# jimmc414/semantic_merge

Measured on AMD Instinct MI355X. Metric: op-log compose+conflict throughput (ops/s), 100M-op logs, 1/2/4/8 GPUs, higher is better.
Workload: dtype u64; 1 GPU; c3: one merge of 100,000,000 ops (100,000,000 per GPU), 1,000,000 symbols, 64 ops/ms, seed 11; n_ops_per_gpu=100000000, n_ops_total=100000000, n_sym=1000000, composed_ops=99989720, conflicts=5140, plan=presorted, parallelism=single GPU

## Files before the change

### include/smx.h

```cpp
#ifndef SMX_H
#define SMX_H

#include <stddef.h>
#include <stdint.h>

#ifdef __cplusplus
extern "C" {
#endif

#define SMX_OK 0
#define SMX_E_ARG (-1)
#define SMX_E_CAPACITY (-2)
#define SMX_E_HIP (-3)
#define SMX_E_WORKSPACE (-4)

#define SMX_KIND_MOVE 0
#define SMX_KIND_RENAME 1
#define SMX_N_KINDS 18
#define SMX_NONE (-1)

typedef struct smx_ops {
  int64_t n_a;
  int64_t n_b;
  int64_t n_sym;
// ... 8 lines not shown
} smx_ops;

typedef struct smx_compose_out {
  int32_t* order;
  int32_t* addr;
  int32_t* file;
  int32_t* ctx;
  int32_t* conflicts;
  int64_t conflict_cap;
  int64_t* counts;
} smx_compose_out;

int smx_compose_workspace_bytes(int64_t n_a, int64_t n_b, int64_t n_sym, size_t* bytes);

int smx_compose(const smx_ops* ops, const smx_compose_out* out, void* workspace,
                size_t workspace_bytes, void* stream);

int smx_compose_async(const smx_ops* ops, const smx_compose_out* out, void* workspace,
                      size_t workspace_bytes, void* stream);
int smx_compose_finish(const smx_ops* ops, const smx_compose_out* out, void* workspace,
                       size_t workspace_bytes, void* stream);

int smx_release_graphs(void* stream);

#define SMX_PLAN_PRESORTED 0
#define SMX_PLAN_SEGMENTED 1
#define SMX_PLAN_RADIX 2
#define SMX_PLAN_RADIX_LO 3
#define SMX_PLAN_PRESORTED_WIDE 4
#define SMX_PLAN_SMALL 5
int smx_last_plan(void);

int64_t smx_set_small_limit(int64_t n);

typedef struct smx_batch {
  int64_t n_merges, n_total, n_sym;
  const int64_t* off;
  const int64_t* n_a;
  const uint8_t* kind; const uint64_t* ts, *oid_hi, *oid_lo;
  const uint32_t* sym; const int32_t* v0, *v1;
  int32_t* order, *addr, *file, *ctx;
  int32_t* conflicts; const int64_t* conf_off;
  int64_t* counts;
  int32_t grid_cap;
} smx_batch;
int smx_compose_batch_workspace_bytes(int64_t n_merges, size_t* bytes);
int smx_compose_batch(const smx_batch* b, void* workspace, size_t workspace_bytes, void* stream);

typedef struct smx_batch_shared {
  int64_t n_merges, n_total, n_sym;
  int64_t n_shared;
  const int64_t* off;
  const uint8_t* kind; const uint64_t* ts, *oid_hi, *oid_lo;
  const uint32_t* sym; const int32_t* v0, *v1;
  int32_t* order, *addr, *file, *ctx;
  int32_t* conflicts; const int64_t* conf_off;
  int64_t* counts;
  int32_t grid_cap;
  int32_t shared_is_b;
} smx_batch_shared;
int smx_compose_batch_shared_workspace_bytes(int64_t n_merges, size_t* bytes);
int smx_compose_batch_shared(const smx_batch_shared* b, void* workspace, size_t workspace_bytes, void* stream);

#define SMX_BATCH_LARGE 1u
int smx_compose_batch_ex_workspace_bytes(int64_t n_merges, int64_t n_total, uint32_t flags, size_t* bytes);
int smx_compose_batch_shared_ex_workspace_bytes(int64_t n_merges, int64_t n_total, int64_t n_shared, uint32_t flags,
// ... 138 lines not shown
```

### semantic_merge_amd/_abi.py

```python
from __future__ import annotations

import ctypes as C

c_i64p = C.POINTER(C.c_int64)


class SmxOps(C.Structure):
    _fields_ = [
        ("n_a", C.c_int64),
        ("n_b", C.c_int64),
        ("n_sym", C.c_int64),
        ("kind", C.c_void_p),
        ("ts", C.c_void_p),
        ("oid_hi", C.c_void_p),
        ("oid_lo", C.c_void_p),
        ("sym", C.c_void_p),
        ("v0", C.c_void_p),
        ("v1", C.c_void_p),
        ("b_gap", C.c_int64),
    ]


class SmxComposeOut(C.Structure):
    _fields_ = [
# ... 177 lines not shown
        ("list", C.c_void_p),
        ("op", C.c_void_p),
        ("value", C.c_void_p),
        ("anchor", C.c_void_p),
        ("t", C.c_void_p),
        ("author", C.c_void_p),
        ("opid_hi", C.c_void_p),
        ("opid_lo", C.c_void_p),
    ]


class SmxRgaOut(C.Structure):
    _fields_ = [
        ("out_value", C.c_void_p),
        ("out_src", C.c_void_p),
        ("out_offsets", C.c_void_p),
        ("counts", C.c_void_p),
        ("out_tomb", C.c_void_p),
    ]


RGA_GROUPED = 1
SCREEN_LARGE = 1
BATCH_LARGE = 1

EXPORTS = (
    "smx_compose_workspace_bytes",
    "smx_compose",
    "smx_compose_async",
    "smx_compose_finish",
    "smx_release_graphs",
    "smx_last_plan",
    "smx_set_small_limit",
    "smx_compose_batch_workspace_bytes",
    "smx_compose_batch",
    "smx_compose_batch_shared_workspace_bytes",
    "smx_compose_batch_shared",
    "smx_compose_batch_ex_workspace_bytes",
    "smx_compose_batch_ex",
    "smx_compose_batch_shared_ex_workspace_bytes",
    "smx_compose_batch_shared_ex",
    "smx_compose_pairs_workspace_bytes",
    "smx_compose_pairs",
    "smx_screen_workspace_bytes",
    "smx_screen",
    "smx_screen_ex_workspace_bytes",
    "smx_screen_ex",
    "smx_screen_candidates_workspace_bytes",
    "smx_screen_candidates",
    "smx_shard_step",
    "smx_shard_range_info",
    "smx_set_profiling",
    "smx_set_profiling_stages",
    "smx_stage_times",
    "smx_stage_name",
    "smx_reset_stage_times",
    "smx_rga_workspace_bytes",
    "smx_rga_replay",
    "smx_rga_replay_ex",
    "smx_last_error",
    "smx_version",
)


def declare(lib: C.CDLL) -> C.CDLL:
    lib.smx_compose_workspace_bytes.argtypes = [C.c_int64, C.c_int64, C.c_int64,
                                                C.POINTER(C.c_size_t)]
    lib.smx_compose_workspace_bytes.restype = C.c_int
    lib.smx_compose.argtypes = [C.POINTER(SmxOps), C.POINTER(SmxComposeOut), C.c_void_p,
                                C.c_size_t, C.c_void_p]
    lib.smx_compose.restype = C.c_int
    for f in ("smx_compose_async", "smx_compose_finish"):
        getattr(lib, f).argtypes = lib.smx_compose.argtypes
        getattr(lib, f).restype = C.c_int
    lib.smx_release_graphs.argtypes = [C.c_void_p]
    lib.smx_release_graphs.restype = C.c_int
    lib.smx_last_plan.argtypes = []
    lib.smx_last_plan.restype = C.c_int
    lib.smx_set_small_limit.argtypes = [C.c_int64]
    lib.smx_set_small_limit.restype = C.c_int64
    if hasattr(lib, "smx_compose_batch"):
        lib.smx_compose_batch_workspace_bytes.argtypes = [C.c_int64, C.POINTER(C.c_size_t)]
        lib.smx_compose_batch_workspace_bytes.restype = C.c_int
        lib.smx_compose_batch.argtypes = [C.POINTER(SmxBatch), C.c_void_p, C.c_size_t, C.c_void_p]
        lib.smx_compose_batch.restype = C.c_int
    if hasattr(lib, "smx_compose_batch_shared"):
        lib.smx_compose_batch_shared_workspace_bytes.argtypes = [C.c_int64, C.POINTER(C.c_size_t)]
        lib.smx_compose_batch_shared_workspace_bytes.restype = C.c_int
        lib.smx_compose_batch_shared.argtypes = [C.POINTER(SmxBatchShared), C.c_void_p, C.c_size_t, C.c_void_p]
        lib.smx_compose_batch_shared.restype = C.c_int
    if hasattr(lib, "smx_compose_batch_ex"):
        lib.smx_compose_batch_ex_workspace_bytes.argtypes = [C.c_int64, C.c_int64, C.c_uint32, C.POINTER(C.c_size_t)]
        lib.smx_compose_batch_ex_workspace_bytes.restype = C.c_int
        lib.smx_compose_batch_ex.argtypes = [C.POINTER(SmxBatch), C.c_void_p, C.c_size_t, C.c_uint32, C.c_void_p]
        lib.smx_compose_batch_ex.restype = C.c_int
        lib.smx_compose_batch_shared_ex_workspace_bytes.argtypes = [C.c_int64, C.c_int64, C.c_int64, C.c_uint32,
                                                                    C.POINTER(C.c_size_t)]
        lib.smx_compose_batch_shared_ex_workspace_bytes.restype = C.c_int
        lib.smx_compose_batch_shared_ex.argtypes = [C.POINTER(SmxBatchShared), C.c_void_p, C.c_size_t, C.c_uint32,
                                                    C.c_void_p]
        lib.smx_compose_batch_shared_ex.restype = C.c_int
    if hasattr(lib, "smx_compose_pairs"):
        lib.smx_compose_pairs_workspace_bytes.argtypes = [C.c_int64, C.c_int64, C.c_int64, C.c_uint32,
                                                          C.POINTER(C.c_size_t)]
        lib.smx_compose_pairs_workspace_bytes.restype = C.c_int
        lib.smx_compose_pairs.argtypes = [C.POINTER(SmxPairs), C.c_void_p, C.c_size_t, C.c_uint32, C.c_void_p]
        lib.smx_compose_pairs.restype = C.c_int
    if hasattr(lib, "smx_screen"):
        lib.smx_screen_workspace_bytes.argtypes = [C.c_int64, C.c_int64, C.c_int64, C.POINTER(C.c_size_t)]
        lib.smx_screen_workspace_bytes.restype = C.c_int
        lib.smx_screen.argtypes = [C.POINTER(SmxScreen), C.c_void_p, C.c_size_t, C.c_void_p]
        lib.smx_screen.restype = C.c_int
    if hasattr(lib, "smx_screen_ex"):
# ... 41 lines not shown
```

### semantic_merge_amd/csrc/smx_compose.hip

```cpp
#include <algorithm>
#include <atomic>
#include <cstring>
#include <mutex>
#include <string>
#include <vector>

#include "smx_sort.h"
#include "smx_window.h"
#include "smx_small.h"
#include "smx_tables.h"


#include "smx_prof.h"

#include "smx_plan.h"
#include "smx_walk.h"

#include "smx_emit.h"


struct Layout {
  size_t off[64];
  size_t total;
};
// ... 243 lines not shown
  if (!tb_geometry(C, &width, &nbk)) return SMX_OK;
  TbArgs A = tb_args(C);
  A.width = (u32)width;
  A.nbk = (u32)nbk;
  A.keep_skip = 1u;
  hipLaunchKernelGGL(k_tb_scatter, dim3((int)SMX_CEIL_DIV((u64)C.n, (u64)TB_TILE)), dim3(TB_NT), 0, C.st, A,
                     C.ws<u32>(B_TBHIST), C.ws<u32>(B_REC));
  HIP_TRY(hipGetLastError());
  return SMX_OK;
}

static int launch_tables(const Ctx& C, void* part_tab, u32 tag, int tagbits, bool* bucketed,
                         bool prescattered = false) {
  hipStream_t st = C.st;
  const i64 n = C.n;
  int4* fin = C.ws<int4>(B_FIN);
  *bucketed = false;
  const i64 n_sym = C.n_sym;
  TbArgs A = tb_args(C);
  u64 width, nbk;
  if (tb_geometry(C, &width, &nbk)) {
    *bucketed = true;
    A.width = (u32)width;
    A.nbk = (u32)nbk;
    const int nblk = (int)SMX_CEIL_DIV((u64)n, (u64)TB_TILE);
    u32* lst = C.ws<u32>(B_TBHIST);
    u32* rec = C.ws<u32>(B_REC);
    if (prescattered) {
      A.keep_skip = 1u;
      hipLaunchKernelGGL(k_tb_unskip, dim3(1024), dim3(BLOCK), 0, st, A, lst, rec, C.ws<u32>(B_SKIPLIST));
    } else {
      hipLaunchKernelGGL(k_tb_scatter, dim3(nblk), dim3(TB_NT), 0, st, A, lst, rec);
    }
    hipLaunchKernelGGL(k_tb_reduce, dim3(nbk), dim3(TBR_NT), 0, st, A, lst, rec, n_sym, fin,
                       PartTab{part_tab, tag, tagbits, C.ws<ComposeMeta>(B_META)});
  } else {
    u32* tabA = C.ws<u32>(B_TABA);
    u32* tabF = C.ws<u32>(B_TABF);
    u32* tabR = C.ws<u32>(B_TABR);
    int rc;
    if ((rc = zero_async(tabA, (size_t)n_sym * 4, st)) || (rc = zero_async(tabF, (size_t)n_sym * 4, st)) ||
        (rc = zero_async(tabR, (size_t)n_sym * 4, st)))
      return rc;
    hipLaunchKernelGGL(k_tab_atomic, dim3(grid_for(n)), dim3(BLOCK), 0, st, A, tabA, tabF, tabR);
    hipLaunchKernelGGL(k_finalize, dim3(grid_for(n_sym)), dim3(BLOCK), 0, st, A, tabA, tabF, tabR, n_sym, fin,
                       PartTab{part_tab, tag, tagbits, C.ws<ComposeMeta>(B_META)});
  }
  HIP_TRY(hipGetLastError());
  return SMX_OK;
}

static int launch_emit(const Ctx& C, bool packable, const smx_shard* sh) {
  hipStream_t st = C.st;
  ComposeMeta* meta = C.ws<ComposeMeta>(B_META);
  const i64 n = C.n;
  EmitArgs E{C.ws<i32>(B_TSRC), C.ws<u32>(B_TSYM), C.ws<u64>(B_SKIPBITS), C.ws<u32>(B_SKIPLIST),
             C.ws<int4>(B_FIN), meta, (u64)n, (u32)(C.n_sym - 1), packable ? 1 : 0, (u64)C.na, C.src_a,
             C.src_b, C.src_map, C.out->order, C.out->addr, C.out->file, C.out->ctx, C.out->counts, sh ? 0 : 1,
             sh ? nullptr : C.hrec, C.hseq};
  const i64 ewaves = SMX_CEIL_DIV(n, (i64)EMIT_WT);
  const bool al16 = ((uintptr_t)C.out->order | (uintptr_t)C.out->addr | (uintptr_t)C.out->file |
                     (uintptr_t)C.out->ctx) % 16 == 0;
  if (al16)
    hipLaunchKernelGGL(k_emit4, dim3(SMX_CEIL_DIV(ewaves, (i64)NWAVES)), dim3(BLOCK), 0, st, E);
  else
    hipLaunchKernelGGL(k_emit, dim3(SMX_CEIL_DIV(ewaves, (i64)NWAVES)), dim3(BLOCK), 0, st, E);
  HIP_TRY(hipGetLastError());
  return SMX_OK;
}

#if SMX_DIAG
static int knob(const char* name, int dflt) {
  const char* v = getenv(name);
  return v && *v ? atoi(v) : dflt;
}
#else
static constexpr int knob(const char*, int dflt) { return dflt; }
#endif

struct SideStream {
  std::mutex mu;
  int dev = -1;
  hipStream_t caller = nullptr;
  hipStream_t s = nullptr;
  hipEvent_t fork = nullptr, join = nullptr;
};
#define SIDE_MAX 256
static std::mutex g_side_mu;
static SideStream* g_side[SIDE_MAX];
static int g_nside = 0;

static int side_stream(hipStream_t caller, SideStream** out) {
  *out = nullptr;
  int dev = 0;
  HIP_TRY(hipGetDevice(&dev));
  std::lock_guard<std::mutex> g(g_side_mu);
  for (int i = 0; i < g_nside; ++i)
    if (g_side[i]->dev == dev && g_side[i]->caller == caller) {
      *out = g_side[i];
      return SMX_OK;
    }
  if (g_nside == SIDE_MAX) return SMX_OK;
  SideStream* S = new SideStream;
  S->dev = dev;
  S->caller = caller;
  int ncu = 0;
  HIP_TRY(hipDeviceGetAttribute(&ncu, hipDeviceAttributeMultiprocessorCount, dev));
  const int k = knob("SMX_SIDE_CUS", 0);
  if (k > 0 && k < ncu) {
    std::vector<uint32_t> mask((size_t)(ncu + 31) / 32, 0u);
    for (int i = 0; i < k; ++i) mask[(size_t)i / 32] |= 1u << (i % 32);
    HIP_TRY(hipExtStreamCreateWithCUMask(&S->s, (uint32_t)mask.size(), mask.data()));
  } else {
    HIP_TRY(hipStreamCreateWithFlags(&S->s, hipStreamNonBlocking));
  }
  const unsigned evf = hipEventDisableTiming | hipEventDisableSystemFence;
  HIP_TRY(hipEventCreateWithFlags(&S->fork, evf));
  HIP_TRY(hipEventCreateWithFlags(&S->join, evf));
  g_side[g_nside++] = S;
  *out = S;
  return SMX_OK;
}

#ifndef SMX_TB_UNSKIP_MAXN
#define SMX_TB_UNSKIP_MAXN (1 << 22)
#endif
#ifndef SMX_TB_OVERLAP_MIN
#define SMX_TB_OVERLAP_MIN (1 << 18)
#endif

static int launch_tail(const Ctx& C) {
  u64 width, nbk;
  const bool geo = tb_geometry(C, &width, &nbk);
  SideStream* S = nullptr;
  if (geo && C.n >= SMX_TB_OVERLAP_MIN && !knob("SMX_TB_SERIAL", 0)) {
    int rc = side_stream(C.st, &S);
    if (rc) return rc;
  }
  std::unique_lock<std::mutex> own;
  int rc;
  hipStream_t st = C.st;
  TbArgs A{};
  u32* lst = C.ws<u32>(B_TBHIST);
  u32* rec = C.ws<u32>(B_REC);
  if (S) {
    own = std::unique_lock<std::mutex>(S->mu);
    A = tb_args(C);
    A.width = (u32)width;
    A.nbk = (u32)nbk;
    A.keep_skip = C.n <= SMX_TB_UNSKIP_MAXN ? 2u : 1u;
    const int nblk = (int)SMX_CEIL_DIV((u64)C.n, (u64)TB_TILE);
    HIP_TRY(hipEventRecord(S->fork, st));
    HIP_TRY(hipStreamWaitEvent(S->s, S->fork, 0));
    hipLaunchKernelGGL(k_tb_scatter, dim3(nblk), dim3(TB_NT), 0, S->s, A, lst, rec);
    HIP_TRY(hipGetLastError());
    HIP_TRY(hipEventRecord(S->join, S->s));
  }
  C.tm->begin(ST_WALK);
  if ((rc = launch_walk(C, nullptr))) {
    if (S) (void)hipStreamWaitEvent(st, S->join, 0);
    return rc;
  }
  C.tm->end(ST_WALK);
  if (S) HIP_TRY(hipStreamWaitEvent(st, S->join, 0));
  C.tm->begin(ST_TABLES);
  bool bucketed = true;
  if (S) {
    if (A.keep_skip == 1u)
      hipLaunchKernelGGL(k_tb_unskip, dim3(1024), dim3(BLOCK), 0, st, A, lst, rec, C.ws<u32>(B_SKIPLIST));
    hipLaunchKernelGGL(k_tb_reduce, dim3(nbk), dim3(TBR_NT), 0, st, A, lst, rec, C.n_sym, C.ws<int4>(B_FIN),
                       PartTab{nullptr, 0u, 0, nullptr});
    HIP_TRY(hipGetLastError());
  } else if ((rc = launch_tables(C, nullptr, 0, 0, &bucketed))) {
    return rc;
  }
  C.tm->end(ST_TABLES);
  C.tm->begin(ST_EMIT);
  if ((rc = launch_emit(C, bucketed, nullptr))) return rc;
  C.tm->end(ST_EMIT);
  return SMX_OK;
}


struct EarlyFail {
  u32* flag_host = nullptr;
  u32* flag_dev = nullptr;
  hipEvent_t ev = nullptr;
};
enum WinLevel { WL_NORMAL, WL_WIDE };
static i64 level_cap(int lv) { return lv == WL_WIDE ? WF_WIDE_CAP : WF_CAP; }
static int first_level(const Ctx& C) { return knob("SMX_FIRST_WIDE", 0) ? WL_WIDE : WL_NORMAL; }
static i64 first_tgt(const Ctx& C) {
  return knob("SMX_WIN_TGT", first_level(C) == WL_WIDE ? WF_WIDE_CAP : WIN_TGT);
}

template <int CAP, int NT, bool DBG, bool MAP, bool RUNS>
static void launch_window_f(const WinArgs& P, hipStream_t st) {
  hipLaunchKernelGGL((k_window_f<CAP, NT, DBG, MAP, RUNS>), dim3(P.W), dim3(NT), 0, st, P);
}
template <int CAP, int NT>
static void launch_window_level(const WinArgs& P, hipStream_t st) {
  if (P.src_map) launch_window_f<CAP, NT, false, true, true>(P, st);
  else launch_window_f<CAP, NT, false, false, true>(P, st);
}

static int launch_presorted_windows(const Ctx& C, i64 W, i64 CM, int level) {
  const bool wide = level == WL_WIDE;
  hipStream_t st = C.st;
  WinArgs P = win_args(C);
  P.cpre = C.ws<u32>(B_CCNT);
  P.CM = CM;
// ... 564 lines not shown
  return entry(ops,
               [&] { return compose_async_impl(ops, out, workspace, workspace_bytes, (hipStream_t)stream, false); });
}

extern "C" int smx_compose_finish(const smx_ops* ops, const smx_compose_out* out, void* workspace,
                                  size_t workspace_bytes, void* stream) {
  return entry(ops, [&] { return compose_finish_impl(ops, out, workspace, workspace_bytes, (hipStream_t)stream); });
}

extern "C" int smx_compose(const smx_ops* ops, const smx_compose_out* out, void* workspace,
                           size_t workspace_bytes, void* stream) {
  return entry(ops, [&] {
    EarlyVerdict ev;
    if (SmallRec* r = small_rec()) {
      ev.hrec = r->d;
      ev.hrec_host = r->h;
      ev.hseq = ++r->seq;
    }
    const int rc = compose_async_impl(ops, out, workspace, workspace_bytes, (hipStream_t)stream, true, &ev);
    return rc ? rc : compose_finish_impl(ops, out, workspace, workspace_bytes, (hipStream_t)stream, &ev);
  });
}

extern "C" int smx_last_plan(void) { return g_plan; }

#ifdef SMALL_STAMPS
extern "C" int smx_diag_small_stamps(uint64_t* host16) {
  HIP_TRY(hipDeviceSynchronize());
  HIP_TRY(hipMemcpyFromSymbol(host16, HIP_SYMBOL(g_small_stamp), 16 * sizeof(u64)));
  return SMX_OK;
}
#endif

extern "C" int64_t smx_set_small_limit(int64_t n) {
  const int64_t v = n < 0 ? 0 : n > SMALL_N ? SMALL_N : n;
  return g_small_max.exchange(v);
}


extern "C" const char* smx_version(void) { return "smx 0.2 gfx950"; }
```

### semantic_merge_amd/csrc/smx_emit.h

```cpp
#pragma once

struct EmitArgs {
  const i32* tsrc;
  const u32* tsym;
  const u64* skipbits;
  const u32* skiplist;
  const int4* fin;
  const ComposeMeta* meta;
  u64 n;
  u32 smax;
  int allow_pack;
  u64 na_loc;
  i64 src_a, src_b;
  const i32* src_map;
  i32* out_order;
  i32* out_addr;
  i32* out_file;
  i32* out_ctx;
  i64* counts;
  int status_none;
  u64* hrec;
  u64 hseq;
};

#define NTLD(p) __builtin_nontemporal_load(p)
#define NTST(v, p) __builtin_nontemporal_store((v), (p))
#ifndef EMIT_WT
#define EMIT_WT 1024
#endif
#ifndef EMIT_B
#define EMIT_B 8
#endif
static_assert(EMIT_WT % (WAVE * EMIT_B) == 0, "a wave's output range is whole batches of steps");

__global__ void __launch_bounds__(BLOCK) k_emit(EmitArgs E) {
  const ComposeMeta* M = E.meta;
  if (blockIdx.x == 0 && threadIdx.x == 0) {
    const bool bad = M->bad_sym != 0;
    E.counts[0] = bad ? -1 : M->f_fail ? -2 : (M->n_move_none && E.status_none) ? -3 : (i64)(E.n - M->n_skip);
    E.counts[1] = bad ? -1 : (i64)M->n_conf;
    if (E.hrec) *E.hrec = E.hseq << 1 | ((bad || M->f_fail || (M->n_move_none && M->kcnt[KMOVE])) ? 1u : 0u);
  }
  if (M->f_fail | M->bad_sym) return;
  const u64 nskip = M->n_skip;
  const u64 nmv = min(M->kcnt[KMOVE], E.n);
  const u64 nP = E.n - nmv;
  const u64 nR = min(M->kcnt[KREN], nP);
  const u64 nout = E.n - nskip, nRk = nR - nskip;
  auto gsrc = [&](i32 j) -> i32 {
    if (E.src_map) return E.src_map[j];
    return (u64)j < E.na_loc ? (i32)(E.src_a + j) : (i32)(E.src_b + ((i64)j - (i64)E.na_loc));
  };
  const FinPack FP = fin_pack_of(M->vbits, E.allow_pack != 0);
  const int lane = threadIdx.x & (WAVE - 1);
  const u64 w0 = (((u64)blockIdx.x * BLOCK + threadIdx.x) / WAVE) * EMIT_WT;
// ... 40 lines not shown
    for (int j = 0; j < EMIT_B; ++j) {
      src[j] = NTLD(&E.tsrc[pp[j]]);
      sy[j] = min(NTLD(&E.tsym[pp[j]]), E.smax);
    }
    int4 F[EMIT_B];
    if (FP.packed) {
      u64 x[EMIT_B];
#pragma unroll
      for (int j = 0; j < EMIT_B; ++j) x[j] = fin_word(FP, E.fin, sy[j]);
#pragma unroll
      for (int j = 0; j < EMIT_B; ++j) F[j] = fin_decode(FP, x[j]);
    } else {
#pragma unroll
      for (int j = 0; j < EMIT_B; ++j) F[j] = E.fin[sy[j]];
    }
#pragma unroll
    for (int j = 0; j < EMIT_B; ++j) {
      const u64 o = ob + (u64)j * WAVE + lane;
      if (o >= nmv && o < nout) {
        const bool ren = o - nmv < nRk;
        NTST(gsrc(src[j]), &E.out_order[o]);
        NTST(F[j].x, &E.out_addr[o]);
        NTST(F[j].y, &E.out_file[o]);
        NTST(ren ? -1 : F[j].z, &E.out_ctx[o]);
      }
    }
  }
}

#define EMIT4_STEPS (EMIT_WT / (4 * WAVE))
typedef u32 ev4u __attribute__((ext_vector_type(4)));
typedef i32 ev4i __attribute__((ext_vector_type(4)));
typedef ev4u __attribute__((aligned(4))) ev4u_a4;
__global__ void __launch_bounds__(BLOCK) k_emit4(EmitArgs E) {
  const ComposeMeta* M = E.meta;
  if (blockIdx.x == 0 && threadIdx.x == 0) {
    const bool bad = M->bad_sym != 0;
    E.counts[0] = bad ? -1 : M->f_fail ? -2 : (M->n_move_none && E.status_none) ? -3 : (i64)(E.n - M->n_skip);
    E.counts[1] = bad ? -1 : (i64)M->n_conf;
    if (E.hrec) *E.hrec = E.hseq << 1 | ((bad || M->f_fail || (M->n_move_none && M->kcnt[KMOVE])) ? 1u : 0u);
  }
  if (M->f_fail | M->bad_sym) return;
  const u64 nskip = M->n_skip;
  const u64 nmv = min(M->kcnt[KMOVE], E.n);
  const u64 nP = E.n - nmv;
  const u64 nR = min(M->kcnt[KREN], nP);
  const u64 nout = E.n - nskip, nRk = nR - nskip;
  auto gsrc = [&](i32 j) -> i32 {
    if (E.src_map) return E.src_map[j];
    return (u64)j < E.na_loc ? (i32)(E.src_a + j) : (i32)(E.src_b + ((i64)j - (i64)E.na_loc));
  };
  const FinPack FP = fin_pack_of(M->vbits, E.allow_pack != 0);
  const int lane = threadIdx.x & (WAVE - 1);
  const u64 w0 = (((u64)blockIdx.x * BLOCK + threadIdx.x) / WAVE) * EMIT_WT;
  if (w0 + EMIT_WT <= nmv || w0 >= nout || nP == 0) return;
  u64 kk = 0;
  {
    const u64 o0 = w0 > nmv ? w0 - nmv : 0;
    if (o0 < nRk) {
      u64 lo = 0, hi = nskip;
      while (lo < hi) {
        const u64 mid = (lo + hi) >> 1;
        if ((u64)E.skiplist[mid] - mid < o0) lo = mid + 1;
        else hi = mid;
      }
      kk = lo;
    }
  }
  u64 pp[EMIT4_STEPS][4];
  bool vec[EMIT4_STEPS];
#pragma unroll
  for (int j = 0; j < EMIT4_STEPS; ++j) {
    const u64 b = w0 + (u64)j * 4 * WAVE;
    const u64 o = b + 4 * (u64)lane;
    u64 add[4] = {0, 0, 0, 0};
    const u64 k0 = kk;
    if (b + 4 * WAVE > nmv && (b > nmv ? b - nmv : 0) < nRk) {
      const u64 ohi = b + 4 * WAVE - 1 - nmv;
      while (kk < nskip) {
        const u64 sj = (u64)(u32)__builtin_amdgcn_readfirstlane((int)E.skiplist[kk]) - kk;
        if (sj > ohi) break;
#pragma unroll
        for (int u = 0; u < 4; ++u) add[u] += (o + u >= nmv ? o + u - nmv : 0) >= sj;
        ++kk;
      }
    }
#pragma unroll
    for (int u = 0; u < 4; ++u) {
      const u64 ou = o + u;
      const u64 op = ou >= nmv ? ou - nmv : 0;
      const bool ok = ou >= nmv && ou < nout;
      pp[j][u] = !ok ? 0 : (op < nRk ? op + k0 + add[u] : op + nskip);
    }
    vec[j] = o >= nmv && o + 3 < nout && pp[j][3] == pp[j][0] + 3;
  }
  i32 src[EMIT4_STEPS][4];
  u32 sy[EMIT4_STEPS][4];
#pragma unroll
  for (int j = 0; j < EMIT4_STEPS; ++j) {
    if (vec[j]) {
      const ev4u s4 = __builtin_nontemporal_load(reinterpret_cast<const ev4u_a4*>(&E.tsrc[pp[j][0]]));
      const ev4u y4 = __builtin_nontemporal_load(reinterpret_cast<const ev4u_a4*>(&E.tsym[pp[j][0]]));
      src[j][0] = (i32)s4.x, src[j][1] = (i32)s4.y, src[j][2] = (i32)s4.z, src[j][3] = (i32)s4.w;
      sy[j][0] = y4.x, sy[j][1] = y4.y, sy[j][2] = y4.z, sy[j][3] = y4.w;
    } else {
#pragma unroll
      for (int u = 0; u < 4; ++u) {
        src[j][u] = NTLD(&E.tsrc[pp[j][u]]);
        sy[j][u] = NTLD(&E.tsym[pp[j][u]]);
      }
    }
#pragma unroll
    for (int u = 0; u < 4; ++u) sy[j][u] = min(sy[j][u], E.smax);
  }
#pragma unroll
  for (int j = 0; j < EMIT4_STEPS; ++j) {
    int4 F[4];
    if (FP.packed) {
      u64 x[4];
#pragma unroll
      for (int u = 0; u < 4; ++u) x[u] = fin_word(FP, E.fin, sy[j][u]);
#pragma unroll
      for (int u = 0; u < 4; ++u) F[u] = fin_decode(FP, x[u]);
    } else {
#pragma unroll
      for (int u = 0; u < 4; ++u) F[u] = E.fin[sy[j][u]];
    }
    const u64 o = w0 + (u64)j * 4 * WAVE + 4 * (u64)lane;
    i32 vo[4], va[4], vf[4], vc[4];
#pragma unroll
    for (int u = 0; u < 4; ++u) {
      const bool ren = o + u >= nmv && o + u - nmv < nRk;
      vo[u] = gsrc(src[j][u]);
      va[u] = F[u].x;
      vf[u] = F[u].y;
      vc[u] = ren ? -1 : F[u].z;
    }
    if (o >= nmv && o + 3 < nout) {
      NTST((ev4i{vo[0], vo[1], vo[2], vo[3]}), reinterpret_cast<ev4i*>(&E.out_order[o]));
      NTST((ev4i{va[0], va[1], va[2], va[3]}), reinterpret_cast<ev4i*>(&E.out_addr[o]));
      NTST((ev4i{vf[0], vf[1], vf[2], vf[3]}), reinterpret_cast<ev4i*>(&E.out_file[o]));
      NTST((ev4i{vc[0], vc[1], vc[2], vc[3]}), reinterpret_cast<ev4i*>(&E.out_ctx[o]));
    } else {
#pragma unroll
      for (int u = 0; u < 4; ++u) {
        if (o + u >= nmv && o + u < nout) {
          E.out_order[o + u] = vo[u];
          E.out_addr[o + u] = va[u];
          E.out_file[o + u] = vf[u];
          E.out_ctx[o + u] = vc[u];
        }
      }
    }
  }
}

__global__ void k_mv_init(const u32* __restrict__ msym, u64 nMv, u64* __restrict__ keys, u32* __restrict__ vals) {
  for (u64 j = (u64)blockIdx.x * BLOCK + threadIdx.x; j < nMv; j += (u64)gridDim.x * BLOCK) {
    keys[j] = msym[j] & SYM_MASK;
    vals[j] = (u32)j;
  }
}

__global__ void k_mv_fix(const u64* __restrict__ keys, const u32* __restrict__ vals, u64 nMv,
                         const u32* __restrict__ msym, const u64* __restrict__ mvpre, u64 n_sym,
                         i32* __restrict__ out_addr, i32* __restrict__ out_file) {
  for (u64 j = (u64)blockIdx.x * BLOCK + threadIdx.x; j < nMv; j += (u64)gridDim.x * BLOCK) {
    if (j != 0 && keys[j - 1] == keys[j]) continue;
    i32 ra = -1, rf = -1;
    if (mvpre && keys[j] < n_sym) {
      const u64 pa = mvpre[keys[j]], pf = mvpre[n_sym + keys[j]];
      if (pa) ra = (i32)(u32)pa - 1;
      if (pf) rf = (i32)(u32)pf - 1;
    }
    for (u64 i = j; i < nMv && keys[i] == keys[j]; ++i) {
      const u32 T = vals[i];
      const u32 f = msym[T];
      if (f & MS_HAS_A) ra = out_addr[T];
      else out_addr[T] = ra;
      if (f & MS_HAS_F) rf = out_file[T];
      else out_file[T] = rf;
    }
  }
}
```

### semantic_merge_amd/csrc/smx_tables.h

```cpp
#pragma once

#include "smx_scan.h"

#define TB_WIDTH 4096
#define TB_MAXBK 1024
#ifndef TB_NT
#define TB_NT 1024
#endif
#define TB_NW (TB_NT / WAVE)
#ifndef TB_ITEMS
#define TB_ITEMS 16
#endif
#ifndef TB_NBK_TGT
#define TB_NBK_TGT 256
#endif
#define TB_TILE (TB_NT * TB_ITEMS)
#define REC_IB (TB_TILE <= (1 << 14) ? 14 : 15)
static_assert(TB_TILE <= (1 << 15), "tile-relative record index is at most 15 bits");
#define REC_IMASK ((1u << REC_IB) - 1u)
#define REC_HAS_A (1u << (REC_IB + 12))
#define REC_HAS_F (1u << (REC_IB + 13))

struct TbArgs {
  const u32* msym;
// ... 167 lines not shown

#define TBR_NT 1024
#ifndef TBR_TK
#define TBR_TK 16
#endif
#ifndef TBR_U
#define TBR_U 2
#endif

struct PartTab {
  void* p;
  u32 tag;
  int tagbits;
  ComposeMeta* meta;
  __device__ __forceinline__ void put(i64 n_sym, i64 s, int va, int vf, int vc) const {
    if (tagbits == 0) {
      u64* part = (u64*)p;
      const u64 tg = (u64)tag << 32;
      part[s] = va >= 0 ? tg | (u32)(va + 1) : 0ull;
      part[n_sym + s] = vf >= 0 ? tg | (u32)(vf + 1) : 0ull;
      part[2 * n_sym + s] = vc >= 0 ? tg | (u32)(vc + 1) : 0ull;
      return;
    }
    u32* part = (u32*)p;
    const u32 vb = 31u - (u32)tagbits, tg = tag << vb, lim = 1u << vb;
    const u32 a1 = (u32)(va + 1), f1 = (u32)(vf + 1), c1 = (u32)(vc + 1);
    if ((a1 | f1 | c1) >= lim) meta->tab_over = 1;
    part[s] = va >= 0 ? tg | (a1 & (lim - 1)) : 0u;
    part[n_sym + s] = vf >= 0 ? tg | (f1 & (lim - 1)) : 0u;
    part[2 * n_sym + s] = vc >= 0 ? tg | (c1 & (lim - 1)) : 0u;
  }
};

__global__ void __launch_bounds__(TBR_NT) k_tb_reduce(TbArgs A0, const u32* __restrict__ lst,
                                                      const u32* __restrict__ rec, i64 n_sym,
                                                      int4* __restrict__ fin, PartTab part) {
  const FinPack FP = fin_pack_of(A0.meta->vbits, true);
  __shared__ u32 tA[TB_WIDTH], tF[TB_WIDTH], tC[TB_WIDTH];
  const TbArgs A = tb_load(A0);
  const u32 b = (u32)xcd_item(blockIdx.x, gridDim.x);
  for (u32 i = threadIdx.x; i < A.width; i += TBR_NT) tA[i] = tF[i] = tC[i] = 0;
  __syncthreads();
  auto put = [&](u32 q, u64 rb) {
    const u32 r1 = (u32)(rb + (q & REC_IMASK)) + 1u;
    const u32 ls = (q >> REC_IB) & 0xfffu;
    if ((u64)(r1 - 1) < A.nMv) {
      if (q & REC_HAS_A) atomicMax(&tA[ls], r1);
      if (q & REC_HAS_F) atomicMax(&tF[ls], r1);
    } else if (A.keep_skip != 2u || !tb_skipped(A, (u64)(r1 - 1) - A.nMv)) {
      atomicMax(&tC[ls], r1);
    }
  };
  const u64 nrec = A.nMv + A.nR;
  const int nt = nrec ? (int)SMX_CEIL_DIV(nrec, (u64)TB_TILE) : 0;
  const int lane = threadIdx.x & (WAVE - 1), wv = threadIdx.x / WAVE;
  const u32 nb1 = A.nbk + 1;
  constexpr int NW = TBR_NT / WAVE;
  auto bounds = [&](int t0, u32* lo, u32* hi) {
    *lo = *hi = 0;
    if (lane < TBR_TK && t0 + lane < nt) {
      const u32* lt = lst + (u64)(t0 + lane) * nb1;
      *lo = lt[b];
      *hi = lt[b + 1];
    }
  };
  u32 lo_n = 0, hi_n = 0;
  bounds(wv * TBR_TK, &lo_n, &hi_n);
  for (int t0 = wv * TBR_TK; t0 < nt; t0 += NW * TBR_TK) {
    const u32 lo = lo_n, hi = hi_n;
    u32 q[TBR_TK][TBR_U];
#pragma unroll
    for (int k = 0; k < TBR_TK; ++k) {
      const u32 lk = __builtin_amdgcn_readlane(lo, k), hk = __builtin_amdgcn_readlane(hi, k);
      const u64 rb = (u64)(t0 + k) * TB_TILE;
#pragma unroll
      for (int u = 0; u < TBR_U; ++u) {
        const u32 i = lk + (u32)lane + (u32)(u * WAVE);
        q[k][u] = i < hk ? __builtin_nontemporal_load(&rec[rb + i]) : ~0u;
      }
    }
    bounds(t0 + NW * TBR_TK, &lo_n, &hi_n);
#pragma unroll
    for (int k = 0; k < TBR_TK; ++k)
#pragma unroll
      for (int u = 0; u < TBR_U; ++u)
        if (q[k][u] != ~0u) put(q[k][u], (u64)(t0 + k) * TB_TILE);
#pragma unroll
    for (int k = 0; k < TBR_TK; ++k) {
      const u32 lk = __builtin_amdgcn_readlane(lo, k), hk = __builtin_amdgcn_readlane(hi, k);
      const u64 rb = (u64)(t0 + k) * TB_TILE;
      for (u32 i = lk + TBR_U * WAVE + (u32)lane; i < hk; i += WAVE) {
        const u32 x = rec[rb + i];
        if (x != REC_DEAD) put(x, rb);
      }
    }
  }
  __syncthreads();
  const u32 s0 = b * A.width;
  for (u32 i = threadIdx.x; i < A.width && (i64)(s0 + i) < n_sym; i += TBR_NT) {
    const u32 a = tA[i], f = tF[i], c = tC[i];
    const int va = a ? A.mv_addr[a - 1] : -1, vf = f ? A.mv_file[f - 1] : -1;
    const int vc = c ? A.Rstr[(u64)(c - 1) - A.nMv] : -1;
    if (part.p) part.put(n_sym, s0 + i, va, vf, vc);
    else fin_put(FP, fin, s0 + i, va, vf, vc);
  }
}

__global__ void k_tab_atomic(TbArgs A0, u32* __restrict__ tabA, u32* __restrict__ tabF, u32* __restrict__ tabR) {
  const TbArgs A = tb_load(A0);
  const u64 nrec = A.nMv + A.nR;
  for (u64 r = (u64)blockIdx.x * BLOCK + threadIdx.x; r < nrec; r += (u64)gridDim.x * BLOCK) {
    u32 s, fl;
    if (!tb_record(A, r, &s, &fl)) continue;
    const u32 r1 = (u32)r + 1u;
    if (r < A.nMv) {
      if (fl & REC_HAS_A) atomicMax(&tabA[s], r1);
      if (fl & REC_HAS_F) atomicMax(&tabF[s], r1);
    } else {
      atomicMax(&tabR[s], r1);
    }
  }
}

__global__ void k_finalize(TbArgs A0, const u32* __restrict__ tabA, const u32* __restrict__ tabF,
                           const u32* __restrict__ tabR, i64 n_sym, int4* __restrict__ fin, PartTab part) {
  const TbArgs A = tb_load(A0);
  for (i64 s = (i64)blockIdx.x * BLOCK + threadIdx.x; s < n_sym; s += (i64)gridDim.x * BLOCK) {
    const u32 a = tabA[s], f = tabF[s], c = tabR[s];
    const int va = a ? A.mv_addr[a - 1] : -1, vf = f ? A.mv_file[f - 1] : -1;
    const int vc = c ? A.Rstr[(u64)(c - 1) - A.nMv] : -1;
    if (part.p) part.put(n_sym, s, va, vf, vc);
    else fin[s] = make_int4(va, vf, vc, 0);
  }
}
```

Baseline: 42.64 billion ops/s.

## Split tail reduce into move and rename phases overlapped with emit

For large merges, the table reduce is split in two. The move-table part runs on the side stream right after scatter and writes a packed addr/file table. The rename part is fused into one kernel that also emits the rename output range, and a second emit kernel handles the remaining range. The aim is to overlap reduce work with emit and shorten the serial tail. The cost is an extra packed table pass, re-reading the move table in the rename phase, and more kernel launches.

```diff
diff --git a/include/smx.h b/include/smx.h
--- a/include/smx.h
+++ b/include/smx.h
@@ -64,6 +64,8 @@
 int smx_last_plan(void);
 
 int64_t smx_set_small_limit(int64_t n);
+
+int64_t smx_set_tail_split_min(int64_t n);
 
 typedef struct smx_batch {
   int64_t n_merges, n_total, n_sym;
diff --git a/semantic_merge_amd/_abi.py b/semantic_merge_amd/_abi.py
--- a/semantic_merge_amd/_abi.py
+++ b/semantic_merge_amd/_abi.py
@@ -233,6 +233,7 @@
     "smx_release_graphs",
     "smx_last_plan",
     "smx_set_small_limit",
+    "smx_set_tail_split_min",
     "smx_compose_batch_workspace_bytes",
     "smx_compose_batch",
     "smx_compose_batch_shared_workspace_bytes",
@@ -280,6 +281,9 @@
     lib.smx_last_plan.restype = C.c_int
     lib.smx_set_small_limit.argtypes = [C.c_int64]
     lib.smx_set_small_limit.restype = C.c_int64
+    if hasattr(lib, "smx_set_tail_split_min"):
+        lib.smx_set_tail_split_min.argtypes = [C.c_int64]
+        lib.smx_set_tail_split_min.restype = C.c_int64
     if hasattr(lib, "smx_compose_batch"):
         lib.smx_compose_batch_workspace_bytes.argtypes = [C.c_int64, C.POINTER(C.c_size_t)]
         lib.smx_compose_batch_workspace_bytes.restype = C.c_int
diff --git a/semantic_merge_amd/csrc/smx_compose.hip b/semantic_merge_amd/csrc/smx_compose.hip
--- a/semantic_merge_amd/csrc/smx_compose.hip
+++ b/semantic_merge_amd/csrc/smx_compose.hip
@@ -299,8 +299,8 @@
     } else {
       hipLaunchKernelGGL(k_tb_scatter, dim3(nblk), dim3(TB_NT), 0, st, A, lst, rec);
     }
-    hipLaunchKernelGGL(k_tb_reduce, dim3(nbk), dim3(TBR_NT), 0, st, A, lst, rec, n_sym, fin,
-                       PartTab{part_tab, tag, tagbits, C.ws<ComposeMeta>(B_META)});
+    hipLaunchKernelGGL(k_tb_reduce<TBM_ALL>, dim3(nbk), dim3(TBR_NT), 0, st, A, lst, rec, n_sym, fin,
+                       (void*)nullptr, PartTab{part_tab, tag, tagbits, C.ws<ComposeMeta>(B_META)});
   } else {
     u32* tabA = C.ws<u32>(B_TABA);
     u32* tabF = C.ws<u32>(B_TABF);
@@ -317,19 +317,26 @@
   return SMX_OK;
 }
 
+static void* af_table(const Ctx& C) { return C.ws<void>(B_TABA); }
+
+static EmitArgs emit_args(const Ctx& C, bool packable, const smx_shard* sh) {
+  return EmitArgs{C.ws<i32>(B_TSRC), C.ws<u32>(B_TSYM), C.ws<u64>(B_SKIPBITS), C.ws<u32>(B_SKIPLIST),
+                  C.ws<int4>(B_FIN), C.ws<ComposeMeta>(B_META), (u64)C.n, (u32)(C.n_sym - 1), packable ? 1 : 0,
+                  (u64)C.na, C.src_a, C.src_b, C.src_map, C.out->order, C.out->addr, C.out->file, C.out->ctx,
+                  C.out->counts, sh ? 0 : 1, sh ? nullptr : C.hrec, C.hseq, nullptr};
+}
+
+static bool emit_aligned(const Ctx& C) {
+  return ((uintptr_t)C.out->order | (uintptr_t)C.out->addr | (uintptr_t)C.out->file | (uintptr_t)C.out->ctx) % 16 ==
+         0;
+}
+
 static int launch_emit(const Ctx& C, bool packable, const smx_shard* sh) {
   hipStream_t st = C.st;
-  ComposeMeta* meta = C.ws<ComposeMeta>(B_META);
-  const i64 n = C.n;
-  EmitArgs E{C.ws<i32>(B_TSRC), C.ws<u32>(B_TSYM), C.ws<u64>(B_SKIPBITS), C.ws<u32>(B_SKIPLIST),
-             C.ws<int4>(B_FIN), meta, (u64)n, (u32)(C.n_sym - 1), packable ? 1 : 0, (u64)C.na, C.src_a,
-             C.src_b, C.src_map, C.out->order, C.out->addr, C.out->file, C.out->ctx, C.out->counts, sh ? 0 : 1,
-             sh ? nullptr : C.hrec, C.hseq};
-  const i64 ewaves = SMX_CEIL_DIV(n, (i64)EMIT_WT);
-  const bool al16 = ((uintptr_t)C.out->order | (uintptr_t)C.out->addr | (uintptr_t)C.out->file |
-                     (uintptr_t)C.out->ctx) % 16 == 0;
-  if (al16)
-    hipLaunchKernelGGL(k_emit4, dim3(SMX_CEIL_DIV(ewaves, (i64)NWAVES)), dim3(BLOCK), 0, st, E);
+  const EmitArgs E = emit_args(C, packable, sh);
+  const i64 ewaves = SMX_CEIL_DIV(C.n, (i64)EMIT_WT);
+  if (emit_aligned(C))
+    hipLaunchKernelGGL(k_emit4<EP_ALL>, dim3(SMX_CEIL_DIV(ewaves, (i64)NWAVES)), dim3(BLOCK), 0, st, E);
   else
     hipLaunchKernelGGL(k_emit, dim3(SMX_CEIL_DIV(ewaves, (i64)NWAVES)), dim3(BLOCK), 0, st, E);
   HIP_TRY(hipGetLastError());
@@ -396,6 +403,11 @@
 #define SMX_TB_OVERLAP_MIN (1 << 18)
 #endif
 
+#ifndef SMX_TB_SPLIT_MIN
+#define SMX_TB_SPLIT_MIN (1 << 23)
+#endif
+static std::atomic<int64_t> g_split_min{SMX_TB_SPLIT_MIN};
+
 static int launch_tail(const Ctx& C) {
   u64 width, nbk;
   const bool geo = tb_geometry(C, &width, &nbk);
@@ -404,6 +416,7 @@
     int rc = side_stream(C.st, &S);
     if (rc) return rc;
   }
+  const bool split = S && C.n >= g_split_min.load() && emit_aligned(C);
   std::unique_lock<std::mutex> own;
   int rc;
   hipStream_t st = C.st;
@@ -420,6 +433,9 @@
     HIP_TRY(hipEventRecord(S->fork, st));
     HIP_TRY(hipStreamWaitEvent(S->s, S->fork, 0));
     hipLaunchKernelGGL(k_tb_scatter, dim3(nblk), dim3(TB_NT), 0, S->s, A, lst, rec);
+    if (split)
+      hipLaunchKernelGGL(k_tb_reduce<TBM_MOVES>, dim3(nbk), dim3(TBR_NT), 0, S->s, A, lst, rec, C.n_sym,
+                         (int4*)nullptr, af_table(C), PartTab{nullptr, 0u, 0, nullptr});
     HIP_TRY(hipGetLastError());
     HIP_TRY(hipEventRecord(S->join, S->s));
   }
@@ -435,15 +451,26 @@
   if (S) {
     if (A.keep_skip == 1u)
       hipLaunchKernelGGL(k_tb_unskip, dim3(1024), dim3(BLOCK), 0, st, A, lst, rec, C.ws<u32>(B_SKIPLIST));
-    hipLaunchKernelGGL(k_tb_reduce, dim3(nbk), dim3(TBR_NT), 0, st, A, lst, rec, C.n_sym, C.ws<int4>(B_FIN),
-                       PartTab{nullptr, 0u, 0, nullptr});
+    if (!split)
+      hipLaunchKernelGGL(k_tb_reduce<TBM_ALL>, dim3(nbk), dim3(TBR_NT), 0, st, A, lst, rec, C.n_sym,
+                         C.ws<int4>(B_FIN), (void*)nullptr, PartTab{nullptr, 0u, 0, nullptr});
     HIP_TRY(hipGetLastError());
   } else if ((rc = launch_tables(C, nullptr, 0, 0, &bucketed))) {
     return rc;
   }
   C.tm->end(ST_TABLES);
   C.tm->begin(ST_EMIT);
-  if ((rc = launch_emit(C, bucketed, nullptr))) return rc;
+  if (split) {
+    EmitArgs E = emit_args(C, true, nullptr);
+    E.af = af_table(C);
+    const i64 ewaves = SMX_CEIL_DIV(C.n, (i64)EMIT_WT);
+    hipLaunchKernelGGL(k_emit4_ren_reduce, dim3((u32)nbk + (u32)SMX_CEIL_DIV(ewaves, (i64)(EMITA_NT / WAVE))),
+                       dim3(EMITA_NT), 0, st, E, A, lst, rec, C.n_sym, C.ws<int4>(B_FIN), af_table(C));
+    hipLaunchKernelGGL(k_emit4<EP_REST>, dim3(SMX_CEIL_DIV(ewaves, (i64)NWAVES)), dim3(BLOCK), 0, st, E);
+    HIP_TRY(hipGetLastError());
+  } else if ((rc = launch_emit(C, bucketed, nullptr))) {
+    return rc;
+  }
   C.tm->end(ST_EMIT);
   return SMX_OK;
 }
@@ -1074,6 +1101,8 @@
 }
 #endif
 
+extern "C" int64_t smx_set_tail_split_min(int64_t n) { return g_split_min.exchange(n < 0 ? SMX_TB_SPLIT_MIN : n); }
+
 extern "C" int64_t smx_set_small_limit(int64_t n) {
   const int64_t v = n < 0 ? 0 : n > SMALL_N ? SMALL_N : n;
   return g_small_max.exchange(v);
diff --git a/semantic_merge_amd/csrc/smx_emit.h b/semantic_merge_amd/csrc/smx_emit.h
--- a/semantic_merge_amd/csrc/smx_emit.h
+++ b/semantic_merge_amd/csrc/smx_emit.h
@@ -21,6 +21,7 @@
   int status_none;
   u64* hrec;
   u64 hseq;
+  const void* af;
 };
 
 #define NTLD(p) __builtin_nontemporal_load(p)
@@ -127,14 +128,20 @@
 typedef u32 ev4u __attribute__((ext_vector_type(4)));
 typedef i32 ev4i __attribute__((ext_vector_type(4)));
 typedef ev4u __attribute__((aligned(4))) ev4u_a4;
-__global__ void __launch_bounds__(BLOCK) k_emit4(EmitArgs E) {
+__device__ __forceinline__ void emit_counts(const EmitArgs& E) {
   const ComposeMeta* M = E.meta;
-  if (blockIdx.x == 0 && threadIdx.x == 0) {
-    const bool bad = M->bad_sym != 0;
-    E.counts[0] = bad ? -1 : M->f_fail ? -2 : (M->n_move_none && E.status_none) ? -3 : (i64)(E.n - M->n_skip);
-    E.counts[1] = bad ? -1 : (i64)M->n_conf;
-    if (E.hrec) *E.hrec = E.hseq << 1 | ((bad || M->f_fail || (M->n_move_none && M->kcnt[KMOVE])) ? 1u : 0u);
-  }
+  const bool bad = M->bad_sym != 0;
+  E.counts[0] = bad ? -1 : M->f_fail ? -2 : (M->n_move_none && E.status_none) ? -3 : (i64)(E.n - M->n_skip);
+  E.counts[1] = bad ? -1 : (i64)M->n_conf;
+  if (E.hrec) *E.hrec = E.hseq << 1 | ((bad || M->f_fail || (M->n_move_none && M->kcnt[KMOVE])) ? 1u : 0u);
+}
+
+#define EP_ALL 0
+#define EP_REN 1
+#define EP_REST 2
+template <int PART>
+__device__ __forceinline__ void emit4_wave(const EmitArgs& E, const u64 wave) {
+  const ComposeMeta* M = E.meta;
   if (M->f_fail | M->bad_sym) return;
   const u64 nskip = M->n_skip;
   const u64 nmv = min(M->kcnt[KMOVE], E.n);
@@ -145,10 +152,13 @@
     if (E.src_map) return E.src_map[j];
     return (u64)j < E.na_loc ? (i32)(E.src_a + j) : (i32)(E.src_b + ((i64)j - (i64)E.na_loc));
   };
-  const FinPack FP = fin_pack_of(M->vbits, E.allow_pack != 0);
+  const FinPack FP = PART == EP_REN ? af_pack_of(M->vbits) : fin_pack_of(M->vbits, E.allow_pack != 0);
+  const void* tab = PART == EP_REN ? E.af : (const void*)E.fin;
+  const u64 olo = PART == EP_REST ? nmv + nRk : nmv;
+  const u64 ohi_p = PART == EP_REN ? nmv + nRk : nout;
   const int lane = threadIdx.x & (WAVE - 1);
-  const u64 w0 = (((u64)blockIdx.x * BLOCK + threadIdx.x) / WAVE) * EMIT_WT;
-  if (w0 + EMIT_WT <= nmv || w0 >= nout || nP == 0) return;
+  const u64 w0 = (olo / EMIT_WT + wave) * EMIT_WT;
+  if (w0 >= ohi_p || nP == 0) return;
   u64 kk = 0;
   {
     const u64 o0 = w0 > nmv ? w0 - nmv : 0;
@@ -184,10 +194,10 @@
     for (int u = 0; u < 4; ++u) {
       const u64 ou = o + u;
       const u64 op = ou >= nmv ? ou - nmv : 0;
-      const bool ok = ou >= nmv && ou < nout;
+      const bool ok = ou >= olo && ou < ohi_p;
       pp[j][u] = !ok ? 0 : (op < nRk ? op + k0 + add[u] : op + nskip);
     }
-    vec[j] = o >= nmv && o + 3 < nout && pp[j][3] == pp[j][0] + 3;
+    vec[j] = o >= olo && o + 3 < ohi_p && pp[j][3] == pp[j][0] + 3;
   }
   i32 src[EMIT4_STEPS][4];
   u32 sy[EMIT4_STEPS][4];
@@ -214,12 +224,12 @@
     if (FP.packed) {
       u64 x[4];
 #pragma unroll
-      for (int u = 0; u < 4; ++u) x[u] = fin_word(FP, E.fin, sy[j][u]);
+      for (int u = 0; u < 4; ++u) x[u] = fin_word(FP, tab, sy[j][u]);
 #pragma unroll
       for (int u = 0; u < 4; ++u) F[u] = fin_decode(FP, x[u]);
     } else {
 #pragma unroll
-      for (int u = 0; u < 4; ++u) F[u] = E.fin[sy[j][u]];
+      for (int u = 0; u < 4; ++u) F[u] = reinterpret_cast<const int4*>(tab)[sy[j][u]];
     }
     const u64 o = w0 + (u64)j * 4 * WAVE + 4 * (u64)lane;
     i32 vo[4], va[4], vf[4], vc[4];
@@ -231,7 +241,7 @@
       vf[u] = F[u].y;
       vc[u] = ren ? -1 : F[u].z;
     }
-    if (o >= nmv && o + 3 < nout) {
+    if (o >= olo && o + 3 < ohi_p) {
       NTST((ev4i{vo[0], vo[1], vo[2], vo[3]}), reinterpret_cast<ev4i*>(&E.out_order[o]));
       NTST((ev4i{va[0], va[1], va[2], va[3]}), reinterpret_cast<ev4i*>(&E.out_addr[o]));
       NTST((ev4i{vf[0], vf[1], vf[2], vf[3]}), reinterpret_cast<ev4i*>(&E.out_file[o]));
@@ -239,7 +249,7 @@
     } else {
 #pragma unroll
       for (int u = 0; u < 4; ++u) {
-        if (o + u >= nmv && o + u < nout) {
+        if (o + u >= olo && o + u < ohi_p) {
           E.out_order[o + u] = vo[u];
           E.out_addr[o + u] = va[u];
           E.out_file[o + u] = vf[u];
@@ -248,6 +258,29 @@
       }
     }
   }
+}
+
+template <int PART>
+__global__ void __launch_bounds__(BLOCK) k_emit4(EmitArgs E) {
+  if (blockIdx.x == 0 && threadIdx.x == 0) emit_counts(E);
+  emit4_wave<PART>(E, ((u64)blockIdx.x * BLOCK + threadIdx.x) / WAVE);
+}
+
+#ifndef EMITA_NT
+#define EMITA_NT 512
+#endif
+__global__ void __launch_bounds__(EMITA_NT) k_emit4_ren_reduce(EmitArgs E, TbArgs A0, const u32* __restrict__ lst,
+                                                               const u32* __restrict__ rec, i64 n_sym,
+                                                               int4* __restrict__ fin, void* __restrict__ af) {
+  __shared__ u32 tC[TB_WIDTH];
+  if (blockIdx.x < A0.nbk) {
+    const TbArgs A = tb_load(A0);
+    const u32 b = (u32)xcd_item(blockIdx.x, A0.nbk);
+    tb_reduce_bucket<TBM_RENAMES, EMITA_NT>(A, b, lst, rec, n_sym, fin, af, PartTab{nullptr, 0u, 0, nullptr},
+                                            nullptr, nullptr, tC);
+    return;
+  }
+  emit4_wave<EP_REN>(E, (u64)(blockIdx.x - A0.nbk) * (EMITA_NT / WAVE) + threadIdx.x / WAVE);
 }
 
 __global__ void k_mv_init(const u32* __restrict__ msym, u64 nMv, u64* __restrict__ keys, u32* __restrict__ vals) {
diff --git a/semantic_merge_amd/csrc/smx_tables.h b/semantic_merge_amd/csrc/smx_tables.h
--- a/semantic_merge_amd/csrc/smx_tables.h
+++ b/semantic_merge_amd/csrc/smx_tables.h
@@ -223,30 +223,47 @@
   }
 };
 
-__global__ void __launch_bounds__(TBR_NT) k_tb_reduce(TbArgs A0, const u32* __restrict__ lst,
-                                                      const u32* __restrict__ rec, i64 n_sym,
-                                                      int4* __restrict__ fin, PartTab part) {
-  const FinPack FP = fin_pack_of(A0.meta->vbits, true);
-  __shared__ u32 tA[TB_WIDTH], tF[TB_WIDTH], tC[TB_WIDTH];
-  const TbArgs A = tb_load(A0);
-  const u32 b = (u32)xcd_item(blockIdx.x, gridDim.x);
-  for (u32 i = threadIdx.x; i < A.width; i += TBR_NT) tA[i] = tF[i] = tC[i] = 0;
+#define TBM_ALL 0
+#define TBM_MOVES 1
+#define TBM_RENAMES 2
+
+__device__ __forceinline__ FinPack af_pack_of(const u32* vbits) {
+  const u32 wa = bit_width32(vbits[0]), wf = bit_width32(vbits[1]);
+  return wa + wf <= 48 ? FinPack{wa, wf, true, true} : FinPack{32u, 32u, true, false};
+}
+
+template <int MODE, int NT>
+__device__ __forceinline__ void tb_reduce_bucket(const TbArgs& A, const u32 b, const u32* __restrict__ lst,
+                                                 const u32* __restrict__ rec, i64 n_sym, void* __restrict__ fin,
+                                                 void* __restrict__ af, const PartTab& part, u32* tA, u32* tF,
+                                                 u32* tC) {
+  constexpr bool MV = MODE != TBM_RENAMES, RN = MODE != TBM_MOVES;
+  const FinPack FP = fin_pack_of(A.meta->vbits, true);
+  const FinPack AP = af_pack_of(A.meta->vbits);
+  for (u32 i = threadIdx.x; i < A.width; i += NT) {
+    if (MV) tA[i] = tF[i] = 0;
+    if (RN) tC[i] = 0;
+  }
   __syncthreads();
   auto put = [&](u32 q, u64 rb) {
     const u32 r1 = (u32)(rb + (q & REC_IMASK)) + 1u;
     const u32 ls = (q >> REC_IB) & 0xfffu;
     if ((u64)(r1 - 1) < A.nMv) {
-      if (q & REC_HAS_A) atomicMax(&tA[ls], r1);
-      if (q & REC_HAS_F) atomicMax(&tF[ls], r1);
-    } else if (A.keep_skip != 2u || !tb_skipped(A, (u64)(r1 - 1) - A.nMv)) {
+      if (MV) {
+        if (q & REC_HAS_A) atomicMax(&tA[ls], r1);
+        if (q & REC_HAS_F) atomicMax(&tF[ls], r1);
+      }
+    } else if (RN && (A.keep_skip != 2u || !tb_skipped(A, (u64)(r1 - 1) - A.nMv))) {
       atomicMax(&tC[ls], r1);
     }
   };
   const u64 nrec = A.nMv + A.nR;
-  const int nt = nrec ? (int)SMX_CEIL_DIV(nrec, (u64)TB_TILE) : 0;
+  const u64 rend = MODE == TBM_MOVES ? A.nMv : nrec;
+  const int nt = rend ? (int)SMX_CEIL_DIV(rend, (u64)TB_TILE) : 0;
+  const int tf = MODE == TBM_RENAMES ? (int)(A.nMv / (u64)TB_TILE) : 0;
   const int lane = threadIdx.x & (WAVE - 1), wv = threadIdx.x / WAVE;
   const u32 nb1 = A.nbk + 1;
-  constexpr int NW = TBR_NT / WAVE;
+  constexpr int NW = NT / WAVE;
   auto bounds = [&](int t0, u32* lo, u32* hi) {
     *lo = *hi = 0;
     if (lane < TBR_TK && t0 + lane < nt) {
@@ -256,8 +273,8 @@
     }
   };
   u32 lo_n = 0, hi_n = 0;
-  bounds(wv * TBR_TK, &lo_n, &hi_n);
-  for (int t0 = wv * TBR_TK; t0 < nt; t0 += NW * TBR_TK) {
+  bounds(tf + wv * TBR_TK, &lo_n, &hi_n);
+  for (int t0 = tf + wv * TBR_TK; t0 < nt; t0 += NW * TBR_TK) {
     const u32 lo = lo_n, hi = hi_n;
     u32 q[TBR_TK][TBR_U];
 #pragma unroll
@@ -288,13 +305,41 @@
   }
   __syncthreads();
   const u32 s0 = b * A.width;
-  for (u32 i = threadIdx.x; i < A.width && (i64)(s0 + i) < n_sym; i += TBR_NT) {
-    const u32 a = tA[i], f = tF[i], c = tC[i];
-    const int va = a ? A.mv_addr[a - 1] : -1, vf = f ? A.mv_file[f - 1] : -1;
-    const int vc = c ? A.Rstr[(u64)(c - 1) - A.nMv] : -1;
-    if (part.p) part.put(n_sym, s0 + i, va, vf, vc);
-    else fin_put(FP, fin, s0 + i, va, vf, vc);
-  }
+  for (u32 i = threadIdx.x; i < A.width && (i64)(s0 + i) < n_sym; i += NT) {
+    int va, vf, vc = -1;
+    if (MV) {
+      const u32 a = tA[i], f = tF[i];
+      va = a ? A.mv_addr[a - 1] : -1;
+      vf = f ? A.mv_file[f - 1] : -1;
+    } else {
+      const int4 m = fin_decode(AP, fin_word(AP, af, s0 + i));
+      va = m.x;
+      vf = m.y;
+    }
+    if (RN) {
+      const u32 c = tC[i];
+      vc = c ? A.Rstr[(u64)(c - 1) - A.nMv] : -1;
+    }
+    if (MODE == TBM_MOVES) {
+      if (AP.p48) fin48_store(af, s0 + i, fin_encode(AP, va, vf, -1));
+      else reinterpret_cast<u64*>(af)[s0 + i] = fin_encode(AP, va, vf, -1);
+    } else if (MODE == TBM_ALL && part.p) {
+      part.put(n_sym, s0 + i, va, vf, vc);
+    } else {
+      fin_put(FP, fin, s0 + i, va, vf, vc);
+    }
+  }
+}
+
+template <int MODE>
+__global__ void __launch_bounds__(TBR_NT) k_tb_reduce(TbArgs A0, const u32* __restrict__ lst,
+                                                      const u32* __restrict__ rec, i64 n_sym,
+                                                      int4* __restrict__ fin, void* __restrict__ af, PartTab part) {
+  __shared__ u32 tA[MODE != TBM_RENAMES ? TB_WIDTH : 1], tF[MODE != TBM_RENAMES ? TB_WIDTH : 1];
+  __shared__ u32 tC[MODE != TBM_MOVES ? TB_WIDTH : 1];
+  const TbArgs A = tb_load(A0);
+  const u32 b = (u32)xcd_item(blockIdx.x, gridDim.x);
+  tb_reduce_bucket<MODE, TBR_NT>(A, b, lst, rec, n_sym, fin, af, part, tA, tF, tC);
 }
 
 __global__ void k_tab_atomic(TbArgs A0, u32* __restrict__ tabA, u32* __restrict__ tabF, u32* __restrict__ tabR) {
```

Result: no change. 42.68 billion ops/s (median of 5 runs) (+0.1%).
